# doughtmw/hmd-ego-pose

Measured on AMD Instinct MI355X. Metric: frames/sec at 256x256 bs16 EfficientPose-phi0; ADD(-S) vs ref, higher is better.
Workload: dtype bf16; 1 GPU; EfficientPose phi=0 256x256 bf16 batch=16 per GPU: forward (stem, MBConv, BiFPN, 5 heads) + box/translation decode; seeded random-init weights, N(0,1) frames resident in HBM; 4 batches of 16 in flight per GPU on 4 HIP streams; phi=0, size=256, batch_per_gpu=16, global_batch=16, parallelism=dp1, batches_in_flight=4, anchors=12276, submission_threads=4

## Files before the change

### hmd_ego_pose_amd/csrc/hep_api.cpp

```cpp
#include <stdio.h>
#include <stdlib.h>
#include <string.h>

#include <math.h>

#include <chrono>
#include <fstream>
#include <memory>

#include "hep.h"
#include "hep_host.h"

using namespace hep;

struct hep_handle { Session s; };

static thread_local std::string g_err;
static int fail(int code, const std::string& msg) { g_err = msg; return code; }
#define HIPRET(x) do { hipError_t e_ = (x); if (e_ != hipSuccess) return fail(HEP_ERR_DEVICE, std::string(#x) + ": " + hipGetErrorString(e_)); } while (0)


static int hep_caught() noexcept {
  try { throw; }
  catch (const std::bad_alloc&) { try { g_err = "out of host memory (std::bad_alloc)"; } catch (...) {} }
// ... 722 lines not shown
  const int prec = o.kind == OP_PW ? (o.pw.fp8 ? 2 : (h->s.dtype ? 1 : 0)) : 0;
  char tmp[128];
  switch (o.kind) {
    case OP_STEM: if (o.stem.mfma) snprintf(tmp, sizeof tmp, "stem_kernel<%s, %d>", t, (o.stem.Cout + 15) / 16);
                  else snprintf(tmp, sizeof tmp, "stem_valu_kernel<%s>", t);
                  break;
    case OP_PW: { const int sev = pw_se_variant(o.pw);
                  const bool w8 = o.pw.nwv == 8 && prec == 0 && o.pw.mode == 2 && o.pw.act != ACT_SWISH && (sev == 0 || sev == 3) && o.pw.NT <= 2;
                  const bool fr = o.pw.frag && prec != 2 && o.pw.MT == 2 && o.pw.NT <= PW_FRAG_MAX_NT && o.pw.mode == 2 && sev >= 1 && o.pw.act != ACT_SWISH;
                  snprintf(tmp, sizeof tmp, fr ? "pw_gemm_kernel<%d, %d, %d, %d, %d, %d, %d, true>" : "pw_gemm_kernel<%d, %d, %d, %d, %d, %d, %d>", prec, o.pw.MT, o.pw.NT, o.pw.mode, o.pw.act == ACT_SWISH ? 1 : 0, sev, (w8 || (fr && o.pw.nwv == 8 && prec == 0 && sev == 3 && o.pw.NT <= 2)) ? 8 : 4); break; }
    case OP_DW: snprintf(tmp, sizeof tmp, "dw_kernel<%s, %d, %d, %d>", t, o.dw.k, o.dw.s, o.dw.TW); break;
    case OP_POOL: snprintf(tmp, sizeof tmp, "pool_kernel<%s>", t); break;
    case OP_PWG: snprintf(tmp, sizeof tmp, "pw_group_kernel<%s>", t); break;
    case OP_CHAIN: snprintf(tmp, sizeof tmp, "chain_kernel<%s, %d>", o.chain.bf16 ? "true" : "false", o.chain.stream_w); break;
    case OP_SE: snprintf(tmp, sizeof tmp, "se_finish_kernel<%s>", t); break;
    case OP_MBF: snprintf(tmp, sizeof tmp, "mbf_kernel<%s, %d, %d, %d, %s, %d>", t, o.mbf.k, o.mbf.s, o.mbf.ts, o.mbf.fp8 ? "true" : "false",
                          o.mbf.has_expand && o.mbf.npass > 1 ? (o.mbf.mp_resident ? 2 : 1) : 0);
                 break;
#ifdef HEP_ALT
    case OP_SBF: snprintf(tmp, sizeof tmp, "sbf_kernel<%s>", t); break;
    case OP_LATE: snprintf(tmp, sizeof tmp, "late_kernel"); break;
    case OP_HEADS: snprintf(tmp, sizeof tmp, "heads_kernel"); break;
#endif
    case OP_XBF: { const int sp = xbf_specialised(o.xbf);
                   snprintf(tmp, sizeof tmp, "xbf_kernel<%s, %d, %d, %d, %d, %d, %d, %d>", t, o.xbf.k, o.xbf.s, o.xbf.toh, o.xbf.tow, o.xbf.NT1, sp ? o.xbf.K1 : 0, sp ? o.xbf.NT2 : 0); break; }
    default: if (o.sep.direct) snprintf(tmp, sizeof tmp, "%s<%s, %d, %s>", o.sep.coop ? "tower_coop_kernel" : "tower_kernel", t, o.sep.C, o.sep.direct == 2 ? "true" : "false");
             else {
               const int mode = o.sep.chain ? 2 : (o.sep.nseg == 1 ? 0 : 1);
               const bool wl = o.sep.bf16 && o.sep.off_wpw && mode != 1;
               if (mode == 0 && sep_w8(o.sep)) snprintf(tmp, sizeof tmp, "sep_kernel<%s, 0, false, true>", t);
               else snprintf(tmp, sizeof tmp, wl ? "sep_kernel<%s, %d, true, false>" : "sep_kernel<%s, %d, false, false>", t, mode);
// ... 93 lines not shown
```

### hmd_ego_pose_amd/csrc/hep_internal.h

```cpp
#pragma once
#include <hip/hip_runtime.h>
#include <stdint.h>

static inline uint32_t rcp_u32(uint32_t d) { return d <= 1 ? 0u : (uint32_t)(0x100000000ull / d) + 1u; }

#define HEP_MAX_SRC 3
#define SEP_MAX_TILES_N 6
#define SEP_MAX_TILES_MAP 24

enum { ACT_NONE = 0, ACT_SWISH = 1, ACT_SIGMOID = 2 };
enum { SRC_SAME = 1, SRC_UP = 2, SRC_DOWN = 3 };

struct StemArgs {
  const float* in; int64_t sn, sc, sh, sw;
  const float* w;
  const float* bias;
  void* out;
  int B, H, W, Ho, Wo, Cout, pad_t, pad_l, bf16;
  int mpw; uint32_t tx_rcp, ho_rcp;
  int mfma;
};

#ifdef HEP_ALT
struct SbfArgs {
// ... 19 lines not shown

struct PwArgs {
  const void* A; const void* W; const float* bias;
  const float* hpart; const float* se_br; const void* se_we ; const float* se_be;
  int se_rows, sq, sqp, se_nimg; float inv_hw;
  int se_from_tensor; const float* se_scale;
  const void* res;
  void* out;
  int M, K, N, tilesN;
  int HW;
  int act, bf16, MT, NT;
  int fp8; const float* wscale; float a_scale;
  int mode;
  int nwv;
  int frag;
  int chunksN; uint32_t chunksN_rcp;
  unsigned long long* trace_buf;
};

#define PWG_MAX 8
struct PwgSeg { const void* A; const void* W; const float* bias; void* out; int HW, K, N, tilesN, blk_begin; };
struct PwgArgs { PwgSeg seg[PWG_MAX]; int nseg, B, bf16, strips_per_image; };

struct DwArgs {
  const void* in; const float* w ; const float* bias; void* out;
  float* hpart;
  const float* se_wr;
  int sq, sqp;
  int B, H, W, C, Ho, Wo, k, s, pad_t, pad_l, act, bf16, TW, blocks_per_image;
  uint32_t cg_magic, sw_magic, c_magic;
// ... 13 lines not shown
  const float* bdw;
  void* out;
  float* hpart;
  const float* se_wr;
  int sq, sqp;
  int B, H, W, Cin, Cexp, Ho, Wo, k, s, pad_t, pad_l, has_expand, bf16;
  int CC;
  int ts;
  int npass, kp;
  int mp_resident;
  uint32_t vk_rcp, kpv_rcp;
  size_t off_e, off_we, off_w, lds_bytes;
  int fp8; const float* we_scale; float a_scale;
  int se_tail; unsigned* tail_counter ; SeFinishArgs tail;
  int out_frag;
  int trace;
  int chunks, tiles_x;
  uint32_t chunks_rcp, tiles_x_rcp, gx_rcp;
};

#define XBF_MAXNT1 3
struct XbfArgs {
  const void* in;
  const float* hpart; int se_rows, sq, sqp; float inv_hw;
  const float* se_br; const void* se_we ; const float* se_be;
  const void* blob;
  int blob_bytes;
  const void* res; void* mid;
  void* out;
  float* hpart_out; const float* se_wr; int sq2, sqp2;
// ... 193 lines not shown
  LossArgs f;
  const float* u;
  float* g_cls; float* g_reg; float* g_tr; float* g_hand;
  int32_t* ws;
};
void launch_losses_backward(const LossGradArgs&, hipStream_t);

void launch_stem(const StemArgs&, hipStream_t);
int stem_uses_mfma(int cout, int force = -1);
void launch_pw(const PwArgs&, hipStream_t);
int pw_se_variant(const PwArgs&);
void launch_pwg(const PwgArgs&, hipStream_t);
void launch_dw(const DwArgs&, hipStream_t);
void launch_pool(const PoolArgs&, hipStream_t);
void launch_mbf(const MbfArgs&, hipStream_t);
size_t mbf_lds_layout(int Cin, int CC, int k, int s, int bf16, int has_expand, int max_inside, int ts, MbfArgs* a, int kp = 0);
int mbf_mp_fits(int CC, int kp, int bf16, int max_inside, int ts);
int mbf_mp_resident(int Cin, int CC, int max_inside, int ts);
int mbf_max_inside(int H, int W, int k, int s, int pad_t, int pad_l, int ts);
int mbf_prepare(void);
void launch_sep(const SepArgs&, hipStream_t);
void launch_tower(const SepArgs&, hipStream_t);
#define TOWER_BIAS_MAX 384
#define TOWER_WLDS_MAX (56 * 1024)
constexpr int tower_hdr_tiles(int C, bool bf16, int cap = 6) {
  if (!bf16) return 12;
  const long es = bf16 ? 2 : 4, wp = C + (bf16 ? 8 : 4), kstep = bf16 ? 32 : 16, ks = (C + kstep - 1) / kstep;
  const long fixed = 9L * C * 4 + 4L * ks * 64 * 16;
  const long room = TOWER_WLDS_MAX < 158L * 1024 - fixed ? TOWER_WLDS_MAX : 158L * 1024 - fixed;
  const long t = room / (16 * wp * es + 64);
  return t < 1 ? 1 : (t > cap ? cap : (int)t);
// ... 17 lines not shown
```

### hmd_ego_pose_amd/csrc/hep_knobs.cpp

```cpp
#include "hep_knobs.h"

#include <stdlib.h>
#include <string.h>

namespace hep {

static void env_int(const char* name, int* v) { if (const char* e = getenv(name)) *v = atoi(e); }

Knobs read_knobs() {
  Knobs k;
  env_int("HEP_LANES", &k.lanes);
  env_int("HEP_CHAIN_STREAM", &k.chain_stream);
  env_int("HEP_TOWER_COOP", &k.tower_coop);
  if (const char* e = getenv("HEP_MBF_MP")) k.mbf_mp = !strcmp(e, "force") ? 3 : (atoi(e) == 2 ? 2 : (atoi(e) != 0 ? 1 : 0));
  env_int("HEP_XBF_GENERIC", &k.xbf_generic);
  env_int("HEP_STEM_MFMA", &k.stem_mfma);
  if (const char* e = getenv("HEP_SE_MAXMB")) k.se_maxmb = atof(e);
  env_int("HEP_PW_FRAG", &k.pw_frag);
  env_int("HEP_SEP_WLDS", &k.sep_wlds);
  env_int("HEP_PLAN_DEBUG", &k.plan_debug);
#ifdef HEP_ALT
  env_int("HEP_PW_NT2", &k.pw_nt2);
  env_int("HEP_PW_MT2", &k.pw_mt2);
  env_int("HEP_PW_NT3", &k.pw_nt3);
  env_int("HEP_PW_WIDE", &k.pw_wide);
  env_int("HEP_PW_W8", &k.pw_w8);
  env_int("HEP_PW_W8_MINK", &k.pw_w8_mink);
  env_int("HEP_SE_TAIL", &k.se_tail);
  env_int("HEP_XBF", &k.xbf);
  env_int("HEP_XBF_MINH", &k.xbf_minh);
  env_int("HEP_XBF_TPW", &k.xbf_tpw);
  if (const char* e = getenv("HEP_MBF")) k.mbf = !strcmp(e, "all") ? 1 : (!strcmp(e, "none") ? 0 : -1);
  env_int("HEP_MBF_MAXH", &k.mbf_maxh);
  if (const char* e = getenv("HEP_MBF_TS")) k.mbf_ts8 = atoi(e) == 8;
  env_int("HEP_MBF_TS16_MAXH", &k.mbf_ts16_maxh);
  env_int("HEP_MBF_CC", &k.mbf_cc);
  env_int("HEP_MBF_MP_RES", &k.mbf_mp_res);
  env_int("HEP_DWLDS", &k.dwlds);
  env_int("HEP_LATE", &k.late);
  env_int("HEP_LATE_G", &k.late_g);
  env_int("HEP_LATE_XCD", &k.late_xcd);
  env_int("HEP_HEADS_FUSED", &k.heads_fused);
  env_int("HEP_SBF", &k.sbf);
  env_int("HEP_TOWER", &k.tower);
  env_int("HEP_CHAIN", &k.chain);
  env_int("HEP_CHAIN_F32", &k.chain_f32);
  env_int("HEP_CHAIN_WGLOBAL", &k.chain_wglobal);
  env_int("HEP_PWG", &k.pwg);
  env_int("HEP_SEP_TS4_MAXHW", &k.sep_ts4_maxhw);
#endif
  return k;
// ... 4 lines not shown
```

### hmd_ego_pose_amd/csrc/hep_knobs.h

```cpp
#pragma once

namespace hep {

struct Knobs {
  int lanes = 1;
  int chain_stream = -1;
  int tower_coop = -1;
  int mbf_mp = 1;
  int xbf_generic = 0;
  int stem_mfma = -1;
  double se_maxmb = 4.0;
  int pw_frag = 1;
  int sep_wlds = 1;
  int plan_debug = 0;
  int pw_nt2 = 2;
  int pw_mt2 = 1;
  int pw_wide = 0;
  int pw_nt3 = 0;
  int pw_w8 = 1;
  int pw_w8_mink = 512;
  int se_tail = 0;
  int xbf = 1;
  int xbf_minh = 64;
  int xbf_tpw = 0;
  int mbf = -1;
  int mbf_maxh = 32;
  int mbf_ts8 = 0;
  int mbf_ts16_maxh = 32;
  int mbf_cc = 64;
  int mbf_mp_res = 0;
  int dwlds = -1;
  int late = 0;
  int late_g = 3;
  int late_xcd = 0;
  int heads_fused = 0;
  int sbf = 0;
  int tower = 1;
  int chain = 2;
  int chain_f32 = 1;
  int chain_wglobal = 1;
  int pwg = 1;
  int sep_ts4_maxhw = 0;
};

// ... 4 lines not shown
```

### hmd_ego_pose_amd/csrc/hep_model.cpp

```cpp
#include <math.h>
#include <cmath>
#include <stdio.h>
#include <stdlib.h>
#include <string.h>

#include <algorithm>
#include <functional>
#include <map>

#include "hep.h"
#include "hep_host.h"
#include "hep_knobs.h"

namespace hep {

static const double kScaling[8][2] = {{1.0, 1.0}, {1.0, 1.1}, {1.1, 1.2}, {1.2, 1.4}, {1.4, 1.8}, {1.6, 2.2}, {1.8, 2.6}, {2.0, 3.1}};
static const int kBackboneOfPhi[9] = {0, 1, 2, 3, 4, 5, 6, 6, 7};
static const int kFpnWidth[9] = {64, 88, 112, 160, 224, 288, 384, 384, 384};
static const int kFpnRepeats[9] = {3, 4, 5, 6, 7, 7, 8, 8, 8};
static const int kHeadDepth[9] = {3, 3, 3, 4, 4, 4, 5, 5, 5};
static const int kStages[7][6] = {{1, 3, 1, 1, 32, 16}, {2, 3, 2, 6, 16, 24}, {2, 5, 2, 6, 24, 40}, {3, 3, 2, 6, 40, 80},
                                  {3, 5, 1, 6, 80, 112}, {4, 5, 2, 6, 112, 192}, {1, 3, 1, 6, 192, 320}};
static const float kBnEps = 1e-3f;
static const float kFusionEps = 1e-4f;
// ... 172 lines not shown
  if (!g || !b || !m || !v) return false;
  out->scale.resize(c); out->shift.resize(c);
  for (int i = 0; i < c; i++) {
    const float s = g->data[i] / sqrtf(v->data[i] + kBnEps);
    out->scale[i] = s; out->shift[i] = b->data[i] - m->data[i] * s;
  }
  return true;
}

struct Ref { int op; int field; int seg; int idx; size_t woff; int tensor; };
enum { F_STEM_W, F_STEM_B, F_STEM_OUT, F_PW_A, F_PW_W, F_PW_B, F_PW_RES, F_PW_OUT, F_DW_IN, F_DW_W, F_DW_B,
       F_DW_OUT, F_DW_PART, F_DW_WR, F_MBF_IN, F_MBF_WE, F_MBF_BE, F_MBF_WDW, F_MBF_BDW, F_MBF_OUT, F_MBF_PART, F_MBF_WR, F_MBF_WESCALE, F_PW_WSCALE, F_PW_SESCALE, F_SE_HPART, F_SE_SCALE, F_SE_BR, F_SE_WE, F_SE_BE, F_PW_HPART, F_PW_SEBR, F_PW_SEWE, F_PW_SEBE, F_POOL_IN, F_POOL_OUT, F_PWG_A, F_PWG_W, F_PWG_B, F_PWG_OUT,
       F_SEG_SRC, F_SEG_WDW, F_SEG_WPW, F_SEG_BIAS, F_SEG_OUT, F_CH_EXT_SRC, F_CH_EXT_STORE, F_CH_NODE_OUT, F_CH_WBLOB,
       F_SBF_WS, F_SBF_BS, F_SBF_WDW, F_SBF_BDW, F_SBF_STEM, F_SBF_OUT, F_SBF_PART, F_SBF_WR,
       F_XBF_IN, F_XBF_HPART, F_XBF_SEBR, F_XBF_SEWE, F_XBF_SEBE, F_XBF_BLOB, F_XBF_RES, F_XBF_MID, F_XBF_OUT, F_XBF_PART, F_XBF_WR,
       F_MBFT_SCALE, F_MBFT_BR, F_MBFT_WE, F_MBFT_BE, F_LATE_IN, F_LATE_BLOB, F_LATE_DS, F_LATE_RES, F_LATE_OUT, F_LATE_HPART, F_HEADS_FEAT, F_HEADS_BLOB, F_HEADS_OUT };

struct Planner {
  Session* s; const Pack& pk; std::string* err; WBuilder wb; bool ok = true;
  std::vector<Ref> refs;
  int ntails = 0;
  const Knobs kn;
  Planner(Session* s_, const Pack& p, std::string* e) : s(s_), pk(p), err(e), kn(s_->knobs) { wb.dtype = s_->dtype; }

  int tensor(const std::string& name, int H, int W, int C, bool f32 = false) {
    TensorDesc t; t.name = name; t.H = H; t.W = W; t.C = C; t.f32 = f32;
    t.bytes_per_image = (size_t)H * W * C * (f32 ? 4 : s->esize());
    s->tensors.push_back(t);
    s->tensor_by_name[name] = (int)s->tensors.size() - 1;
    return (int)s->tensors.size() - 1;
  }
// ... 355 lines not shown
    }
    if (boundary) {
    } else if (CC) {
      if (!b.expand) CC = std::min(CC, b.cexp);
      nblk = ((Ho + ts - 1) / ts) * ((Wo + ts - 1) / ts) * ((b.cexp + CC - 1) / CC);
      snprintf(nm, sizeof nm, "b%d.se_hpart", i);
      part_t = tensor(nm, 1, nblk, sqp, true);
      snprintf(nm, sizeof nm, "b%d.front", i);
      const int op = new_op(OP_MBF, nm);
      Op& o = s->ops[op];
      MbfArgs& m = o.mbf; memset(&m, 0, sizeof m);
      m.H = Hin; m.W = Win; m.Cin = b.cin; m.Cexp = b.cexp; m.Ho = Ho; m.Wo = Wo; m.k = b.k; m.s = b.stride;
      m.pad_t = pt; m.pad_l = pl; m.has_expand = b.expand; m.bf16 = s->dtype; m.CC = CC; m.sq = b.se; m.sqp = sqp; m.ts = ts;
      m.npass = npass; m.kp = kp;
      m.mp_resident = npass > 1 && mbf_mp_resident(b.cin, CC, max_in, ts) && kn.mbf_mp_res != 0;
      mbf_lds_layout(b.cin, CC, b.k, b.stride, s->dtype, b.expand, max_in, ts, &m, kp);
      wref(op, F_MBF_WR, wr_off);
      if (b.expand) {
        const PackTensor* w = get(p + "._expand_conv.conv.weight", {b.cexp, b.cin, 1, 1});
        BnFold bn0; if (!fold_bn(pk, p + "._bn0", b.cexp, &bn0, err)) ok = false;
        if (!ok) return -1;
        const int rows = (b.cexp + 15) / 16 * 16;
        std::vector<float> wf((size_t)rows * b.cin, 0.f);
        for (int n = 0; n < b.cexp; n++) for (int k = 0; k < b.cin; k++) wf[(size_t)n * b.cin + k] = w->data[(size_t)n * b.cin + k] * bn0.scale[n];
        if (s->dtype == 2) {
          std::vector<float> sc;
          wref(op, F_MBF_WE, wb.put_fp8(wf, rows, b.cin, (b.cin + 15) & ~15, &sc)); wref(op, F_MBF_WESCALE, wb.put_f32(sc));
          m.fp8 = 1; m.a_scale = 1.f;
        } else wref(op, F_MBF_WE, wb.put_typed(wf));
        wref(op, F_MBF_BE, wb.put_f32(bn0.shift));
      }
// ... 878 lines not shown
      else if (r.tensor <= -2) { const int k = -(r.tensor + 2); ptr = s->d_out[k] + (size_t)lane * s->lane_batch * s->num_anchors * s->out_k(k); }
      else ptr = s->d_weights + r.woff;
      switch (r.field) {
        case F_STEM_W: o.stem.w = (const float*)ptr; break;
        case F_STEM_B: o.stem.bias = (const float*)ptr; break;
        case F_STEM_OUT: o.stem.out = ptr; break;
        case F_PW_A: o.pw.A = ptr; break;
        case F_PW_W: o.pw.W = ptr; break;
        case F_PW_B: o.pw.bias = (const float*)ptr; break;
        case F_PW_HPART: o.pw.hpart = (const float*)ptr; break;
        case F_PW_SEBR: o.pw.se_br = (const float*)ptr; break;
        case F_PW_SEWE: o.pw.se_we = ptr; break;
        case F_PW_SEBE: o.pw.se_be = (const float*)ptr; break;
        case F_PW_RES: o.pw.res = ptr; break;
        case F_PW_OUT: o.pw.out = ptr; break;
        case F_DW_IN: o.dw.in = ptr; break;
        case F_DW_W: o.dw.w = (const float*)ptr; break;
        case F_DW_B: o.dw.bias = (const float*)ptr; break;
        case F_DW_OUT: o.dw.out = ptr; break;
        case F_DW_PART: o.dw.hpart = (float*)ptr; break;
        case F_DW_WR: o.dw.se_wr = (const float*)ptr; break;
        case F_MBF_IN: o.mbf.in = ptr; break;
        case F_MBF_WE: o.mbf.we = ptr; break;
        case F_MBF_BE: o.mbf.be = (const float*)ptr; break;
        case F_MBF_WDW: o.mbf.wdw = (const float*)ptr; break;
        case F_MBF_BDW: o.mbf.bdw = (const float*)ptr; break;
        case F_MBF_OUT: o.mbf.out = ptr; break;
        case F_MBF_PART: o.mbf.hpart = (float*)ptr; o.mbf.tail.hpart = (const float*)ptr; break;
        case F_MBFT_SCALE: o.mbf.tail.scale = (float*)ptr; break;
        case F_MBFT_BR: o.mbf.tail.br = (const float*)ptr; break;
        case F_MBFT_WE: o.mbf.tail.we = ptr; break;
        case F_MBFT_BE: o.mbf.tail.be = (const float*)ptr; break;
        case F_MBF_WR: o.mbf.se_wr = (const float*)ptr; break;
        case F_MBF_WESCALE: o.mbf.we_scale = (const float*)ptr; break;
        case F_PW_WSCALE: o.pw.wscale = (const float*)ptr; break;
        case F_PW_SESCALE: o.pw.se_scale = (const float*)ptr; break;
        case F_SE_HPART: o.se.hpart = (const float*)ptr; break;
// ... 84 lines not shown
```

### hmd_ego_pose_amd/csrc/k_mbf.hip

```cpp
#include <stddef.h>
#include <stdio.h>
#include <stdlib.h>

#include <algorithm>

#include <type_traits>

#include "hep_dev.h"
#include "hep_internal.h"
#include "se_finish.h"


#ifdef HEP_MBF_TRACE
__device__ unsigned long long* g_mbf_trace = nullptr;
#ifdef HEP_MBF_TRACE_A
#define MSTAMP(i) do { if ((i) == 0 || (i) == 6) stamps[i] = __builtin_amdgcn_s_memrealtime(); } while (0)
#define XSTAMP(i) do { stamps[i] = __builtin_amdgcn_s_memrealtime(); } while (0)
#else
#define MSTAMP(i) do { stamps[i] = __builtin_amdgcn_s_memrealtime(); } while (0)
#define XSTAMP(i)
#endif
#else
#define MSTAMP(i)
#define XSTAMP(i)
#endif


template <bool BF16, int KS, int S, int TS, bool F8, int MP>
__global__ __launch_bounds__(TS == 16 ? 1024 : 512) void mbf_kernel(MbfArgs a) {
  constexpr int MBF_THREADS = TS == 16 ? 1024 : 512, MBF_WAVES = MBF_THREADS / 64;
  typedef Vec8<BF16> V;
  typedef typename V::elem T;
  typedef typename std::conditional<BF16, u32x4, f32x4>::type raw_t;
  constexpr int KSTEP = BF16 ? 32 : 16, KLANE = BF16 ? 8 : 4, PAD = BF16 ? 8 : 4;
  constexpr int PW = (TS - 1) * S + KS;
  constexpr int PIN = PW * PW;
  extern __shared__ __attribute__((aligned(16))) unsigned char smem[];
  HEP_POISON(smem, a.lds_bytes);
#ifdef HEP_MBF_TRACE
  unsigned long long stamps[8] = {0, 0, 0, 0, 0, 0, 0, 0};
  MSTAMP(0);
#endif
  const int lane = threadIdx.x & 63, wave = __builtin_amdgcn_readfirstlane(threadIdx.x >> 6);
  const int r = lane & 15, g = lane >> 4;
// ... 38 lines not shown
    const bool ok = tap < KS * KS && c4 < cv;
    wv[j] = *reinterpret_cast<const f32x4*>(wdw_g + (ok ? (uint32_t)(tap * a.Cexp + c4 * 4) : 0u));
  }
  const int bi = threadIdx.x;
  const bool b_dw = bi < cv, b_ex = a.has_expand && bi >= 64 && bi - 64 < cv;
  const f32x4 bv = *reinterpret_cast<const f32x4*>((b_ex ? a.be : a.bdw) + c0 + (b_dw || b_ex ? (uint32_t)(bi & 63) * 4 : 0u));
  auto park_weights = [&]() {
#pragma unroll
    for (int j = 0; j < NDW; j++) {
      const int i = threadIdx.x + j * MBF_THREADS, tap = i >> cvsh, c4 = i & ((1 << cvsh) - 1);
      if (tap < KS * KS && c4 < cv) *reinterpret_cast<f32x4*>(wdw_s + tap * a.CC + c4 * 4) = wv[j];
    }
    if (b_dw) *reinterpret_cast<f32x4*>(bdw_s + bi * 4) = bv;
    else if (b_ex) *reinterpret_cast<f32x4*>(be_s + (bi - 64) * 4) = bv;
  };
  {
    constexpr int NB = BF16 ? 8 : 4;
    constexpr int VB = 8 * (int)sizeof(T);
    const int vecs = a.has_expand ? K >> 3 : cc >> 3;
    const unsigned char* in_b = reinterpret_cast<const unsigned char*>(a.in) + (int64_t)b * a.H * a.W * K * (int)sizeof(T);
    const int vsh = vecs <= 1 ? 0 : 32 - __builtin_clz(vecs - 1);
    const int v = threadIdx.x & ((1 << vsh) - 1), row0 = threadIdx.x >> vsh, rstride = MBF_THREADS >> vsh;
    if constexpr (MP != 0) {
      const int Kp = a.kp, npass = a.npass, n_wrows = ntiles * 16;
      const int pvecs = Kp >> 3;
      const int pvsh = pvecs <= 1 ? 0 : 32 - __builtin_clz(pvecs - 1);
      const int pv = threadIdx.x & ((1 << pvsh) - 1), prow0 = threadIdx.x >> pvsh, prs = MBF_THREADS >> pvsh;
      constexpr int NIW = TS == 16 ? 1 : 2, NIP = TS == 16 ? 2 : 3;
      const unsigned char* w_b = reinterpret_cast<const unsigned char*>(a.we) + (int64_t)c0 * K * (int)sizeof(T);
      const int pix0 = (iy0 + r0) * a.W + ix0 + q0;
// ... 170 lines not shown
          const uint32_t off = (uint32_t)((pix0 + ri * a.W + (m - ri * wi)) * K) * (uint32_t)sizeof(T) + (uint32_t)(v * VB);
          const unsigned char* src = in_b + (vok && mm < n_in ? off : 0u);
          p0[j] = *reinterpret_cast<const raw_t*>(src); if (!BF16) p1[j] = *reinterpret_cast<const raw_t*>(src + 16);
        }
      };
      auto store_p = [&](int base) {
#pragma unroll
        for (int j = 0; j < NH; j++) {
          const int m = base + j * rstride + row0;
          if (vok && m < n_in) {
            raw_t* d = reinterpret_cast<raw_t*>(a_s + m * KP + v * 8);
            d[0] = p0[j]; if (!BF16) d[1] = p1[j];
          }
        }
      };
      issue_w(0); issue_p(0);
      XSTAMP(2); park_weights(); XSTAMP(3);
      store_w(0); store_p(0);
      for (int base = rstride * NH; base < n_wrows; base += rstride * NH) { issue_w(base); store_w(base); }
      for (int base = rstride * NH; base < n_in; base += rstride * NH) { issue_p(base); store_p(base); }
    } else {
      for (int base = 0; base < PIN; base += rstride * NB) {
        raw_t x0[NB], x1[NB];
        bool inside[NB];
#pragma unroll
        for (int j = 0; j < NB; j++) {
          const int p = base + j * rstride + row0, ty = p / PW, gy = iy0 + ty, gx = ix0 + p - ty * PW;
          inside[j] = p < PIN && v < vecs && gy >= 0 && gy < a.H && gx >= 0 && gx < a.W;
          const uint32_t off = (uint32_t)((gy * a.W + gx) * K + c0) * (uint32_t)sizeof(T) + (uint32_t)(v * VB);
          const unsigned char* src = in_b + (inside[j] ? off : 0u);
          x0[j] = *reinterpret_cast<const raw_t*>(src); if (!BF16) x1[j] = *reinterpret_cast<const raw_t*>(src + 16);
        }
        if (base == 0) { XSTAMP(2); park_weights(); XSTAMP(3); }
#pragma unroll
        for (int j = 0; j < NB; j++) {
// ... 4 lines not shown
          }
        }
      }
    }
  }
  if constexpr (MP == 0) {
  MSTAMP(1); XSTAMP(4);
  __syncthreads();
  MSTAMP(2); XSTAMP(5);
  }

  if (MP == 0 && a.has_expand) {
    const int mpairs = (n_in + 31) >> 5;
    const int ntsh = ntiles <= 1 ? 0 : 32 - __builtin_clz(ntiles - 1);
    constexpr int KSMAX = BF16 ? 6 : 12;
    if (!F8 && ksteps <= KSMAX && (1 << ntsh) <= MBF_WAVES) {
      const int nt = wave & ((1 << ntsh) - 1), grp = wave >> ntsh, ngrp = MBF_WAVES >> ntsh;
      const int n = nt * 16 + 4 * g;
      if (nt < ntiles) {
        raw_t wfr[KSMAX];
        const T* wrow = w_s + (nt * 16 + r) * KP;
#pragma unroll
        for (int ks = 0; ks < KSMAX; ks++) {
          const bool kok = ks < ksteps && ks * KSTEP + KLANE * g < K;
          wfr[ks] = *reinterpret_cast<const raw_t*>(wrow + (kok ? ks * KSTEP + KLANE * g : 0));
          if (!kok) wfr[ks] = raw_t{};
        }
        const f32x4 bias = *reinterpret_cast<const f32x4*>(be_s + min(n, cc - 4));
        const int mtiles = (n_in + 15) >> 4;
        for (int mt = grp; mt < mtiles; mt += 2 * ngrp) {
// ... 241 lines not shown
      __syncthreads();
      if (*flag) se_finish_body<BF16, MBF_THREADS, true>(a.tail, b, 0, a.tail.C, threadIdx.x, reinterpret_cast<float*>(smem) + 32);
    }
#endif
  }
#ifdef HEP_MBF_TRACE
  MSTAMP(6);
  if (g_mbf_trace && a.trace && lane == 0) {
    unsigned long long* o = g_mbf_trace + ((size_t)(b * gridDim.x + bxl) * MBF_WAVES + wave) * 8;
    for (int i = 0; i < 7; i++) o[i] = stamps[i];
    o[7] = __builtin_amdgcn_s_getreg((4 << 0) | (0 << 6) | (31 << 11));
  }
#endif
}

#ifdef HEP_MBF_TRACE
extern "C" int hep_dbg_mbf_trace(unsigned long long* host, int max_waves, int enable) {
  static unsigned long long* buf = nullptr;
  const size_t cap = (size_t)1 << 21;
  if (!buf) { if (hipMalloc((void**)&buf, cap * 8) != hipSuccess) return -1; hipMemset(buf, 0, cap * 8); }
  unsigned long long* p = enable ? buf : nullptr;
  hipMemcpyToSymbol(HIP_SYMBOL(g_mbf_trace), &p, sizeof p);
  if (host) { hipDeviceSynchronize(); hipMemcpy(host, buf, (size_t)max_waves * 64, hipMemcpyDeviceToHost); }
  return (int)(cap / 8);
}
#endif

int mbf_max_inside(int H, int W, int k, int s, int pad_t, int pad_l, int ts) {
  const int pw = (ts - 1) * s + k;
  auto span = [&](int n, int pad) {
    const int no = (n + s - 1) / s;
    int best = 0;
    for (int t0 = 0; t0 < no; t0 += ts) {
      const int i0 = t0 * s - pad, lo = std::max(0, -i0), hi = std::min(pw, n - i0);
      best = std::max(best, hi - lo);
    }
    return best;
  };
  return span(H, pad_t) * span(W, pad_l);
}

int mbf_threads(int ts) { return ts == 16 ? 1024 : 512; }

size_t mbf_lds_layout(int Cin, int CC, int k, int s, int bf16, int has_expand, int max_inside, int ts, MbfArgs* a, int kp) {
  const size_t es = bf16 ? 2 : 4, pad = bf16 ? 8 : 4;
  const size_t pw = (size_t)(ts - 1) * s + k, pin = pw * pw;
  const size_t arows = (((size_t)std::min<int>(max_inside, (int)pin) + 31) / 32) * 32;
  const bool mp = has_expand && kp > 0 && kp < Cin;
  const size_t kcols = mp ? (size_t)kp : (size_t)Cin;
  size_t in_bytes = has_expand ? arows * (kcols + pad) * es : 0;
  in_bytes = std::max(in_bytes, mp && ts == 16 ? (size_t)0 : (size_t)mbf_threads(ts) * 9 * 4);
  in_bytes = (in_bytes + 15) & ~(size_t)15;
  const size_t e_bytes = (std::max(pin * (CC + pad) * es, (size_t)16 * CC * 4) + 15) & ~(size_t)15;
  const size_t w_bytes = (size_t)(k * k + 2) * CC * 4;
  const size_t we_bytes = has_expand ? (((size_t)CC * (kcols + pad) * es + 15) & ~(size_t)15) : 0;
  if (a) { a->off_e = in_bytes; a->off_we = in_bytes + e_bytes; a->off_w = a->off_we + we_bytes; a->lds_bytes = a->off_w + w_bytes; }
  return in_bytes + e_bytes + we_bytes + w_bytes;
}

int mbf_mp_fits(int CC, int kp, int bf16, int max_inside, int ts) {
  const int threads = mbf_threads(ts), waves = threads / 64, kstep = bf16 ? 32 : 16;
  if (kp <= 0 || kp % kstep != 0 || kp / kstep > 3) return 0;
  int vp = 1; while (vp < kp / 8) vp <<= 1;
  const int prs = threads / vp, niw = ts == 16 ? 1 : 2, nip = ts == 16 ? 2 : 3;
  const int ntiles = (CC + 15) / 16; int np2 = 1; while (np2 < ntiles) np2 <<= 1;
  if (np2 > waves) return 0;
  const int ngrp = waves / np2, mtiles = (max_inside + 15) / 16, maxmt = ts == 16 ? 7 : 5;
  return ntiles * 16 <= niw * prs && max_inside <= nip * prs && (mtiles + ngrp - 1) / ngrp <= maxmt;
}
int mbf_mp_resident(int Cin, int CC, int max_inside, int ts) {
  const long items = (long)(((CC + 15) / 16) * 16 + max_inside) * (Cin / 8);
  return Cin % 8 == 0 && items <= 6L * mbf_threads(ts);
}

template <bool BF16, int KS, int S, int TS>
static int prep_one() {
  int rc = hipFuncSetAttribute(reinterpret_cast<const void*>(mbf_kernel<BF16, KS, S, TS, false, 0>), hipFuncAttributeMaxDynamicSharedMemorySize, 159 * 1024) == hipSuccess ? 0 : -1;
  rc |= hipFuncSetAttribute(reinterpret_cast<const void*>(mbf_kernel<BF16, KS, S, TS, false, 1>), hipFuncAttributeMaxDynamicSharedMemorySize, 159 * 1024) == hipSuccess ? 0 : -1;
  rc |= hipFuncSetAttribute(reinterpret_cast<const void*>(mbf_kernel<BF16, KS, S, TS, false, 2>), hipFuncAttributeMaxDynamicSharedMemorySize, 159 * 1024) == hipSuccess ? 0 : -1;
#ifdef HEP_WITH_FP8
  if constexpr (BF16) rc |= hipFuncSetAttribute(reinterpret_cast<const void*>(mbf_kernel<true, KS, S, TS, true, 0>), hipFuncAttributeMaxDynamicSharedMemorySize, 159 * 1024) == hipSuccess ? 0 : -1;
#endif
  return rc;
}
int mbf_prepare(void) {
  return prep_one<true, 3, 1, 8>() | prep_one<true, 3, 2, 8>() | prep_one<true, 5, 1, 8>() | prep_one<true, 5, 2, 8>() |
         prep_one<false, 3, 1, 8>() | prep_one<false, 3, 2, 8>() | prep_one<false, 5, 1, 8>() | prep_one<false, 5, 2, 8>() |
         prep_one<true, 3, 1, 16>() | prep_one<true, 5, 1, 16>() | prep_one<false, 3, 1, 16>() | prep_one<false, 5, 1, 16>();
}

template <bool BF16, bool F8, int MP>
static void launch_mbf_t(const MbfArgs& a, dim3 grid, hipStream_t s) {
  if (a.ts == 16) {
    if (a.k == 3) hipLaunchKernelGGL((mbf_kernel<BF16, 3, 1, 16, F8, MP>), grid, dim3(1024), a.lds_bytes, s, a);
    else hipLaunchKernelGGL((mbf_kernel<BF16, 5, 1, 16, F8, MP>), grid, dim3(1024), a.lds_bytes, s, a);
  }
  else if (a.k == 3 && a.s == 1) hipLaunchKernelGGL((mbf_kernel<BF16, 3, 1, 8, F8, MP>), grid, dim3(512), a.lds_bytes, s, a);
  else if (a.k == 3 && a.s == 2) hipLaunchKernelGGL((mbf_kernel<BF16, 3, 2, 8, F8, MP>), grid, dim3(512), a.lds_bytes, s, a);
  else if (a.k == 5 && a.s == 1) hipLaunchKernelGGL((mbf_kernel<BF16, 5, 1, 8, F8, MP>), grid, dim3(512), a.lds_bytes, s, a);
  else hipLaunchKernelGGL((mbf_kernel<BF16, 5, 2, 8, F8, MP>), grid, dim3(512), a.lds_bytes, s, a);
}
void launch_mbf(const MbfArgs& a_, hipStream_t s) {
  MbfArgs a = a_;
#ifdef HEP_MBF_TRACE
  {
    static const char* sel = getenv("HEP_MBF_TRACE_SEL");
    int c = 0, h = 0;
    if (sel) sscanf(sel, "%d,%d", &c, &h);
    a.trace = !sel || (a.Cexp == c && a.H == h);
  }
#endif
  const int tiles = ((a.Wo + a.ts - 1) / a.ts) * ((a.Ho + a.ts - 1) / a.ts), chunks = (a.Cexp + a.CC - 1) / a.CC;
  dim3 grid(tiles * chunks, a.B);
  a.chunks = chunks; a.tiles_x = (a.Wo + a.ts - 1) / a.ts;
  a.chunks_rcp = rcp_u32(chunks); a.tiles_x_rcp = rcp_u32(a.tiles_x); a.gx_rcp = rcp_u32(grid.x);
#ifdef HEP_WITH_FP8
  if (a.bf16 && a.fp8) { launch_mbf_t<true, true, 0>(a, grid, s); return; }
#endif
  const int mp = a.has_expand && a.npass > 1 ? (a.mp_resident ? 2 : 1) : 0;
  a.vk_rcp = rcp_u32((uint32_t)std::max(1, a.Cin >> 3)); a.kpv_rcp = rcp_u32((uint32_t)std::max(1, a.kp >> 3));
  if (a.bf16) { if (mp == 2) launch_mbf_t<true, false, 2>(a, grid, s); else if (mp == 1) launch_mbf_t<true, false, 1>(a, grid, s); else launch_mbf_t<true, false, 0>(a, grid, s); }
  else { if (mp == 2) launch_mbf_t<false, false, 2>(a, grid, s); else if (mp == 1) launch_mbf_t<false, false, 1>(a, grid, s); else launch_mbf_t<false, false, 0>(a, grid, s); }
}
```

### hmd_ego_pose_amd/csrc/k_pw_impl.h

```cpp
#include "hep_dev.h"
#include "hep_internal.h"

#pragma once
#include <type_traits>
#ifndef HEP_PW_UF32
#define HEP_PW_UF32 2
#endif

template <bool BF16> struct Frag;
template <> struct Frag<true> { typedef u32x4 raw; static constexpr int KSTEP = 32, KLANE = 8; };
template <> struct Frag<false> { typedef f32x4 raw; static constexpr int KSTEP = 16, KLANE = 4; };

template <int PREC, int MT, int NT>
struct Step {
  typename Frag<PREC != 0>::raw a[MT];
  typename std::conditional<PREC == 2, u32x2, typename Frag<PREC != 0>::raw>::type w[NT];
};

#ifdef HEP_PW_TRACE
extern unsigned long long* g_pw_trace_host;
#define PSTAMP(i) do { stamps[i] = __builtin_amdgcn_s_memrealtime(); } while (0)
#else
#define PSTAMP(i)
#endif
// ... 322 lines not shown
      float v[4];
#pragma unroll
      for (int q = 0; q < 4; q++) { const float x = F8 ? fmaf(acc[i][j][q], ws[q], b[q]) : acc[i][j][q] + b[q]; v[q] = ACT == ACT_SWISH ? swish_t<BF16>(x) : x; }
      const int64_t o = (int64_t)mrow[i] * a.N + n;
      if (R) {
        float rr[4];
        if constexpr (HOIST) {
          const res_t rv = res_h[i][j >> 2];
          if constexpr (BF16) { rr[0] = __uint_as_float(rv[0] << 16); rr[1] = __uint_as_float(rv[0] & 0xffff0000u); rr[2] = __uint_as_float(rv[1] << 16); rr[3] = __uint_as_float(rv[1] & 0xffff0000u); }
          else { rr[0] = rv[0]; rr[1] = rv[1]; rr[2] = rv[2]; rr[3] = rv[3]; }
        } else V::load4(R, o, rr);
#pragma unroll
        for (int q = 0; q < 4; q++) v[q] += rr[q];
      }
      V::store4(a.out, o, v);
    }
  }
#ifdef HEP_PW_TRACE
  PSTAMP(5);
  if (a.trace_buf && lane == 0 && wave < 4) {
    unsigned long long* o = a.trace_buf + ((size_t)blockIdx.x * 4 + wave) * 8;
    for (int i = 0; i < 6; i++) o[i] = stamps[i];
  }
#endif
}

template <int PREC, int MT, int MODE>
static void launch_nt(const PwArgs& a, dim3 grid, hipStream_t s) {
  const size_t lds = a.sq > 0 ? ((size_t)a.se_nimg * a.K + a.sqp + 256 + a.sqp) * sizeof(float) : 0;
  const int sev = pw_se_variant(a);
// ... 52 lines not shown
```

Before: 56450 frames/s.

## Feed MBConv expand GEMM from producer-written MFMA fragment-ordered activations

The producing pointwise GEMM now also writes its bf16 output in MFMA fragment order to a second tensor. Matching MBConv fronts (stride 1, single pass, whole-image tiles, Cin up to 192) then load their A operand straight from global memory into registers instead of staging input patches in LDS. The aim is to skip the LDS staging and shrink LDS use. The cost is a second output write and extra HBM traffic in the producer.

```diff
diff --git a/hmd_ego_pose_amd/csrc/hep_api.cpp b/hmd_ego_pose_amd/csrc/hep_api.cpp
--- a/hmd_ego_pose_amd/csrc/hep_api.cpp
+++ b/hmd_ego_pose_amd/csrc/hep_api.cpp
@@ -760,7 +760,8 @@
     case OP_PWG: snprintf(tmp, sizeof tmp, "pw_group_kernel<%s>", t); break;
     case OP_CHAIN: snprintf(tmp, sizeof tmp, "chain_kernel<%s, %d>", o.chain.bf16 ? "true" : "false", o.chain.stream_w); break;
     case OP_SE: snprintf(tmp, sizeof tmp, "se_finish_kernel<%s>", t); break;
-    case OP_MBF: snprintf(tmp, sizeof tmp, "mbf_kernel<%s, %d, %d, %d, %s, %d>", t, o.mbf.k, o.mbf.s, o.mbf.ts, o.mbf.fp8 ? "true" : "false",
+    case OP_MBF: if (o.mbf.a_frag) { snprintf(tmp, sizeof tmp, "mbf_afrag_kernel<%d, %d>", o.mbf.k, o.mbf.ts); break; }
+                 snprintf(tmp, sizeof tmp, "mbf_kernel<%s, %d, %d, %d, %s, %d>", t, o.mbf.k, o.mbf.s, o.mbf.ts, o.mbf.fp8 ? "true" : "false",
                           o.mbf.has_expand && o.mbf.npass > 1 ? (o.mbf.mp_resident ? 2 : 1) : 0);
                  break;
 #ifdef HEP_ALT
diff --git a/hmd_ego_pose_amd/csrc/hep_internal.h b/hmd_ego_pose_amd/csrc/hep_internal.h
--- a/hmd_ego_pose_amd/csrc/hep_internal.h
+++ b/hmd_ego_pose_amd/csrc/hep_internal.h
@@ -57,6 +57,7 @@
   int mode;
   int nwv;
   int frag;
+  void* out_frag;
   int chunksN; uint32_t chunksN_rcp;
   unsigned long long* trace_buf;
 };
@@ -100,6 +101,7 @@
   int fp8; const float* we_scale; float a_scale;
   int se_tail; unsigned* tail_counter ; SeFinishArgs tail;
   int out_frag;
+  int a_frag; const void* in_frag;
   int trace;
   int chunks, tiles_x;
   uint32_t chunks_rcp, tiles_x_rcp, gx_rcp;
@@ -323,7 +325,8 @@
 void launch_dw(const DwArgs&, hipStream_t);
 void launch_pool(const PoolArgs&, hipStream_t);
 void launch_mbf(const MbfArgs&, hipStream_t);
-size_t mbf_lds_layout(int Cin, int CC, int k, int s, int bf16, int has_expand, int max_inside, int ts, MbfArgs* a, int kp = 0);
+size_t mbf_lds_layout(int Cin, int CC, int k, int s, int bf16, int has_expand, int max_inside, int ts, MbfArgs* a, int kp = 0, int a_frag = 0);
+int mbf_afrag_supported(int H, int W, int Cin, int k, int s, int ts, int bf16);
 int mbf_mp_fits(int CC, int kp, int bf16, int max_inside, int ts);
 int mbf_mp_resident(int Cin, int CC, int max_inside, int ts);
 int mbf_max_inside(int H, int W, int k, int s, int pad_t, int pad_l, int ts);
diff --git a/hmd_ego_pose_amd/csrc/hep_knobs.cpp b/hmd_ego_pose_amd/csrc/hep_knobs.cpp
--- a/hmd_ego_pose_amd/csrc/hep_knobs.cpp
+++ b/hmd_ego_pose_amd/csrc/hep_knobs.cpp
@@ -35,6 +35,7 @@
   if (const char* e = getenv("HEP_MBF_TS")) k.mbf_ts8 = atoi(e) == 8;
   env_int("HEP_MBF_TS16_MAXH", &k.mbf_ts16_maxh);
   env_int("HEP_MBF_CC", &k.mbf_cc);
+  env_int("HEP_MBF_AFRAG", &k.mbf_afrag);
   env_int("HEP_MBF_MP_RES", &k.mbf_mp_res);
   env_int("HEP_DWLDS", &k.dwlds);
   env_int("HEP_LATE", &k.late);
diff --git a/hmd_ego_pose_amd/csrc/hep_knobs.h b/hmd_ego_pose_amd/csrc/hep_knobs.h
--- a/hmd_ego_pose_amd/csrc/hep_knobs.h
+++ b/hmd_ego_pose_amd/csrc/hep_knobs.h
@@ -28,6 +28,7 @@
   int mbf_ts8 = 0;
   int mbf_ts16_maxh = 32;
   int mbf_cc = 64;
+  int mbf_afrag = 1;
   int mbf_mp_res = 0;
   int dwlds = -1;
   int late = 0;
diff --git a/hmd_ego_pose_amd/csrc/hep_model.cpp b/hmd_ego_pose_amd/csrc/hep_model.cpp
--- a/hmd_ego_pose_amd/csrc/hep_model.cpp
+++ b/hmd_ego_pose_amd/csrc/hep_model.cpp
@@ -210,7 +210,7 @@
        F_SEG_SRC, F_SEG_WDW, F_SEG_WPW, F_SEG_BIAS, F_SEG_OUT, F_CH_EXT_SRC, F_CH_EXT_STORE, F_CH_NODE_OUT, F_CH_WBLOB,
        F_SBF_WS, F_SBF_BS, F_SBF_WDW, F_SBF_BDW, F_SBF_STEM, F_SBF_OUT, F_SBF_PART, F_SBF_WR,
        F_XBF_IN, F_XBF_HPART, F_XBF_SEBR, F_XBF_SEWE, F_XBF_SEBE, F_XBF_BLOB, F_XBF_RES, F_XBF_MID, F_XBF_OUT, F_XBF_PART, F_XBF_WR,
-       F_MBFT_SCALE, F_MBFT_BR, F_MBFT_WE, F_MBFT_BE, F_LATE_IN, F_LATE_BLOB, F_LATE_DS, F_LATE_RES, F_LATE_OUT, F_LATE_HPART, F_HEADS_FEAT, F_HEADS_BLOB, F_HEADS_OUT };
+       F_PW_OUTFRAG, F_MBF_INFRAG, F_MBFT_SCALE, F_MBFT_BR, F_MBFT_WE, F_MBFT_BE, F_LATE_IN, F_LATE_BLOB, F_LATE_DS, F_LATE_RES, F_LATE_OUT, F_LATE_HPART, F_HEADS_FEAT, F_HEADS_BLOB, F_HEADS_OUT };
 
 struct Planner {
   Session* s; const Pack& pk; std::string* err; WBuilder wb; bool ok = true;
@@ -596,7 +596,19 @@
       m.pad_t = pt; m.pad_l = pl; m.has_expand = b.expand; m.bf16 = s->dtype; m.CC = CC; m.sq = b.se; m.sqp = sqp; m.ts = ts;
       m.npass = npass; m.kp = kp;
       m.mp_resident = npass > 1 && mbf_mp_resident(b.cin, CC, max_in, ts) && kn.mbf_mp_res != 0;
-      mbf_lds_layout(b.cin, CC, b.k, b.stride, s->dtype, b.expand, max_in, ts, &m, kp);
+      int frag_src = -1;
+      if (kn.mbf_afrag != 0 && b.expand && npass <= 1 && mbf_afrag_supported(Hin, Win, b.cin, b.k, b.stride, ts, s->dtype))
+        for (const Ref& r : refs) if (r.field == F_PW_OUT && r.tensor == x && s->ops[r.op].kind == OP_PW && s->ops[r.op].pw.bf16 == 1) frag_src = r.op;
+      if (frag_src >= 0) {
+        const int kpad = (b.cin + 31) & ~31;
+        const int ft = tensor(s->tensors[x].name + ".frag", Hin, Win, kpad);
+        s->tensors[ft].C_logical = b.cin; s->tensors[ft].frag = true;
+        tref(frag_src, F_PW_OUTFRAG, ft, true); tref(op, F_MBF_INFRAG, ft, false);
+        s->ops[frag_src].act_bytes_per_image += (double)Hin * Win * kpad * es();
+        m.a_frag = 1;
+      }
+      if (kn.plan_debug) fprintf(stderr, "libhep plan: block %d front: activation operand %s\n", i, m.a_frag ? "from global fragments" : "staged in LDS");
+      mbf_lds_layout(b.cin, CC, b.k, b.stride, s->dtype, b.expand, max_in, ts, &m, kp, m.a_frag);
       wref(op, F_MBF_WR, wr_off);
       if (b.expand) {
         const PackTensor* w = get(p + "._expand_conv.conv.weight", {b.cexp, b.cin, 1, 1});
@@ -1505,6 +1517,7 @@
         case F_PW_SEBE: o.pw.se_be = (const float*)ptr; break;
         case F_PW_RES: o.pw.res = ptr; break;
         case F_PW_OUT: o.pw.out = ptr; break;
+        case F_PW_OUTFRAG: o.pw.out_frag = ptr; break;
         case F_DW_IN: o.dw.in = ptr; break;
         case F_DW_W: o.dw.w = (const float*)ptr; break;
         case F_DW_B: o.dw.bias = (const float*)ptr; break;
@@ -1512,6 +1525,7 @@
         case F_DW_PART: o.dw.hpart = (float*)ptr; break;
         case F_DW_WR: o.dw.se_wr = (const float*)ptr; break;
         case F_MBF_IN: o.mbf.in = ptr; break;
+        case F_MBF_INFRAG: o.mbf.in_frag = ptr; break;
         case F_MBF_WE: o.mbf.we = ptr; break;
         case F_MBF_BE: o.mbf.be = (const float*)ptr; break;
         case F_MBF_WDW: o.mbf.wdw = (const float*)ptr; break;
diff --git a/hmd_ego_pose_amd/csrc/k_mbf.hip b/hmd_ego_pose_amd/csrc/k_mbf.hip
--- a/hmd_ego_pose_amd/csrc/k_mbf.hip
+++ b/hmd_ego_pose_amd/csrc/k_mbf.hip
@@ -26,8 +26,9 @@
 #endif
 
 
-template <bool BF16, int KS, int S, int TS, bool F8, int MP>
-__global__ __launch_bounds__(TS == 16 ? 1024 : 512) void mbf_kernel(MbfArgs a) {
+template <bool BF16, int KS, int S, int TS, bool F8, int MP, bool AF>
+__device__ __forceinline__ void mbf_body(const MbfArgs& a) {
+  static_assert(!AF || (BF16 && S == 1 && !F8 && MP == 0), "fragment-ordered A operand: bf16 single-pass stride-1 fronts only");
   constexpr int MBF_THREADS = TS == 16 ? 1024 : 512, MBF_WAVES = MBF_THREADS / 64;
   typedef Vec8<BF16> V;
   typedef typename V::elem T;
@@ -96,6 +97,11 @@
     if (b_dw) *reinterpret_cast<f32x4*>(bdw_s + bi * 4) = bv;
     else if (b_ex) *reinterpret_cast<f32x4*>(be_s + (bi - 64) * 4) = bv;
   };
+  constexpr int AF_KS = 6;
+  constexpr int AF_MT = TS * TS / 16;
+  constexpr int AF_NTW = 4 * AF_MT / MBF_WAVES;
+  const int af_mt = wave & (AF_MT - 1), af_nt0 = (wave / AF_MT) * AF_NTW;
+  raw_t afr[AF ? AF_KS : 1];
   {
     constexpr int NB = BF16 ? 8 : 4;
     constexpr int VB = 8 * (int)sizeof(T);
@@ -296,11 +302,23 @@
           }
         }
       };
+      if constexpr (AF) {
+        const raw_t* fr = reinterpret_cast<const raw_t*>(a.in_frag) + ((size_t)(b * AF_MT + af_mt) * ksteps) * 64 + lane;
+        issue_w(0);
+#pragma unroll
+        for (int ks = 0; ks < AF_KS; ks++) afr[ks] = fr[min(ks, ksteps - 1) * 64];
+        XSTAMP(2); park_weights(); XSTAMP(3);
+        store_w(0);
+        for (int base = rstride * NH; base < n_wrows; base += rstride * NH) { issue_w(base); store_w(base); }
+#pragma unroll
+        for (int ks = 0; ks < AF_KS; ks++) if (ks >= ksteps || ks * KSTEP + KLANE * g >= K) afr[ks] = raw_t{};
+      } else {
       issue_w(0); issue_p(0);
       XSTAMP(2); park_weights(); XSTAMP(3);
       store_w(0); store_p(0);
       for (int base = rstride * NH; base < n_wrows; base += rstride * NH) { issue_w(base); store_w(base); }
       for (int base = rstride * NH; base < n_in; base += rstride * NH) { issue_p(base); store_p(base); }
+      }
     } else {
       for (int base = 0; base < PIN; base += rstride * NB) {
         raw_t x0[NB], x1[NB];
@@ -335,6 +353,44 @@
     const int mpairs = (n_in + 31) >> 5;
     const int ntsh = ntiles <= 1 ? 0 : 32 - __builtin_clz(ntiles - 1);
     constexpr int KSMAX = BF16 ? 6 : 12;
+    if constexpr (AF) {
+      const int m = af_mt * 16 + r;
+      const int p = (r0 + m / TS) * PW + q0 + (m % TS);
+#pragma unroll
+      for (int j = 0; j < AF_NTW; j += 2) {
+        const int nta = af_nt0 + j, ntb = nta + 1;
+        if (nta < ntiles) {
+          const bool hasb = ntb < ntiles;
+          const T* wra = w_s + (nta * 16 + r) * KP;
+          const T* wrb = w_s + ((hasb ? ntb : nta) * 16 + r) * KP;
+          const int na = nta * 16 + 4 * g, nb = ntb * 16 + 4 * g;
+          f32x4 acc0 = *reinterpret_cast<const f32x4*>(be_s + min(na, cc - 4)), acc1 = *reinterpret_cast<const f32x4*>(be_s + min(nb, cc - 4));
+#pragma unroll
+          for (int ks = 0; ks < AF_KS; ks++) {
+            if (ks < ksteps) {
+              const bool kok = ks * KSTEP + KLANE * g < K;
+              const int ko = kok ? ks * KSTEP + KLANE * g : 0;
+              raw_t w0 = *reinterpret_cast<const raw_t*>(wra + ko), w1 = *reinterpret_cast<const raw_t*>(wrb + ko);
+              if (!kok) { w0 = raw_t{}; w1 = raw_t{}; }
+              acc0 = __builtin_amdgcn_mfma_f32_16x16x32_bf16(__builtin_bit_cast(bf16x8, w0), __builtin_bit_cast(bf16x8, afr[ks]), acc0, 0, 0, 0);
+              acc1 = __builtin_amdgcn_mfma_f32_16x16x32_bf16(__builtin_bit_cast(bf16x8, w1), __builtin_bit_cast(bf16x8, afr[ks]), acc1, 0, 0, 0);
+            }
+          }
+#pragma unroll
+          for (int half = 0; half < 2; half++) {
+            const int n = half ? nb : na;
+            if ((half == 0 || hasb) && n < cc) {
+              const f32x4 acc = half ? acc1 : acc0;
+              float v[4];
+#pragma unroll
+              for (int q = 0; q < 4; q++) v[q] = acc[q];
+              swish_n<BF16, 4>(v);
+              V::store4(e_s, (int64_t)p * EP + n, v);
+            }
+          }
+        }
+      }
+    } else
     if (!F8 && ksteps <= KSMAX && (1 << ntsh) <= MBF_WAVES) {
       const int nt = wave & ((1 << ntsh) - 1), grp = wave >> ntsh, ngrp = MBF_WAVES >> ntsh;
       const int n = nt * 16 + 4 * g;
@@ -606,6 +662,11 @@
 #endif
 }
 
+template <bool BF16, int KS, int S, int TS, bool F8, int MP>
+__global__ __launch_bounds__(TS == 16 ? 1024 : 512) void mbf_kernel(MbfArgs a) { mbf_body<BF16, KS, S, TS, F8, MP, false>(a); }
+template <int KS, int TS>
+__global__ __launch_bounds__(TS == 16 ? 1024 : 512) void mbf_afrag_kernel(MbfArgs a) { mbf_body<true, KS, 1, TS, false, 0, true>(a); }
+
 #ifdef HEP_MBF_TRACE
 extern "C" int hep_dbg_mbf_trace(unsigned long long* host, int max_waves, int enable) {
   static unsigned long long* buf = nullptr;
@@ -634,14 +695,14 @@
 
 int mbf_threads(int ts) { return ts == 16 ? 1024 : 512; }
 
-size_t mbf_lds_layout(int Cin, int CC, int k, int s, int bf16, int has_expand, int max_inside, int ts, MbfArgs* a, int kp) {
+size_t mbf_lds_layout(int Cin, int CC, int k, int s, int bf16, int has_expand, int max_inside, int ts, MbfArgs* a, int kp, int a_frag) {
   const size_t es = bf16 ? 2 : 4, pad = bf16 ? 8 : 4;
   const size_t pw = (size_t)(ts - 1) * s + k, pin = pw * pw;
   const size_t arows = (((size_t)std::min<int>(max_inside, (int)pin) + 31) / 32) * 32;
   const bool mp = has_expand && kp > 0 && kp < Cin;
   const size_t kcols = mp ? (size_t)kp : (size_t)Cin;
-  size_t in_bytes = has_expand ? arows * (kcols + pad) * es : 0;
-  in_bytes = std::max(in_bytes, mp && ts == 16 ? (size_t)0 : (size_t)mbf_threads(ts) * 9 * 4);
+  size_t in_bytes = has_expand && !a_frag ? arows * (kcols + pad) * es : 0;
+  in_bytes = std::max(in_bytes, (mp || a_frag) && ts == 16 ? (size_t)0 : (size_t)mbf_threads(ts) * 9 * 4);
   in_bytes = (in_bytes + 15) & ~(size_t)15;
   const size_t e_bytes = (std::max(pin * (CC + pad) * es, (size_t)16 * CC * 4) + 15) & ~(size_t)15;
   const size_t w_bytes = (size_t)(k * k + 2) * CC * 4;
@@ -665,6 +726,14 @@
   return Cin % 8 == 0 && items <= 6L * mbf_threads(ts);
 }
 
+int mbf_afrag_supported(int H, int W, int Cin, int k, int s, int ts, int bf16) {
+  return bf16 == 1 && s == 1 && (k == 3 || k == 5) && (ts == 8 || ts == 16) && H == ts && W == ts && Cin % 8 == 0 && Cin <= 192;
+}
+
+template <int KS, int TS>
+static int prep_af() {
+  return hipFuncSetAttribute(reinterpret_cast<const void*>(mbf_afrag_kernel<KS, TS>), hipFuncAttributeMaxDynamicSharedMemorySize, 159 * 1024) == hipSuccess ? 0 : -1;
+}
 template <bool BF16, int KS, int S, int TS>
 static int prep_one() {
   int rc = hipFuncSetAttribute(reinterpret_cast<const void*>(mbf_kernel<BF16, KS, S, TS, false, 0>), hipFuncAttributeMaxDynamicSharedMemorySize, 159 * 1024) == hipSuccess ? 0 : -1;
@@ -678,7 +747,8 @@
 int mbf_prepare(void) {
   return prep_one<true, 3, 1, 8>() | prep_one<true, 3, 2, 8>() | prep_one<true, 5, 1, 8>() | prep_one<true, 5, 2, 8>() |
          prep_one<false, 3, 1, 8>() | prep_one<false, 3, 2, 8>() | prep_one<false, 5, 1, 8>() | prep_one<false, 5, 2, 8>() |
-         prep_one<true, 3, 1, 16>() | prep_one<true, 5, 1, 16>() | prep_one<false, 3, 1, 16>() | prep_one<false, 5, 1, 16>();
+         prep_one<true, 3, 1, 16>() | prep_one<true, 5, 1, 16>() | prep_one<false, 3, 1, 16>() | prep_one<false, 5, 1, 16>() |
+         prep_af<3, 8>() | prep_af<5, 8>() | prep_af<3, 16>() | prep_af<5, 16>();
 }
 
 template <bool BF16, bool F8, int MP>
@@ -709,6 +779,11 @@
 #ifdef HEP_WITH_FP8
   if (a.bf16 && a.fp8) { launch_mbf_t<true, true, 0>(a, grid, s); return; }
 #endif
+  if (a.a_frag) {
+    if (a.ts == 16) { if (a.k == 3) hipLaunchKernelGGL((mbf_afrag_kernel<3, 16>), grid, dim3(1024), a.lds_bytes, s, a); else hipLaunchKernelGGL((mbf_afrag_kernel<5, 16>), grid, dim3(1024), a.lds_bytes, s, a); }
+    else { if (a.k == 3) hipLaunchKernelGGL((mbf_afrag_kernel<3, 8>), grid, dim3(512), a.lds_bytes, s, a); else hipLaunchKernelGGL((mbf_afrag_kernel<5, 8>), grid, dim3(512), a.lds_bytes, s, a); }
+    return;
+  }
   const int mp = a.has_expand && a.npass > 1 ? (a.mp_resident ? 2 : 1) : 0;
   a.vk_rcp = rcp_u32((uint32_t)std::max(1, a.Cin >> 3)); a.kpv_rcp = rcp_u32((uint32_t)std::max(1, a.kp >> 3));
   if (a.bf16) { if (mp == 2) launch_mbf_t<true, false, 2>(a, grid, s); else if (mp == 1) launch_mbf_t<true, false, 1>(a, grid, s); else launch_mbf_t<true, false, 0>(a, grid, s); }
diff --git a/hmd_ego_pose_amd/csrc/k_pw_impl.h b/hmd_ego_pose_amd/csrc/k_pw_impl.h
--- a/hmd_ego_pose_amd/csrc/k_pw_impl.h
+++ b/hmd_ego_pose_amd/csrc/k_pw_impl.h
@@ -360,6 +360,13 @@
         for (int q = 0; q < 4; q++) v[q] += rr[q];
       }
       V::store4(a.out, o, v);
+      if constexpr (BF16) {
+        if (a.out_frag) {
+          const int kstN = (a.N + 31) >> 5, m = mrow[i];
+          const int64_t unit = (int64_t)((m >> 4) * kstN + (n >> 5)) * 64 + ((n & 31) >> 3) * 16 + (m & 15);
+          V::store4(a.out_frag, unit * 8 + (n & 7), v);
+        }
+      }
     }
   }
 #ifdef HEP_PW_TRACE
```

After: 56890 frames/s, median of 6. About the same (+0.8%).
